# daviyan5/ninpol

Hardware: AMD Instinct MI355X
Metric: Mnodes/s interpolated (GLS, 10M-cell hex mesh) + achieved HBM GB/s vs peak (higher is better)
Workload: dtype f64

## Files before the change

### ninpol_amd/csrc/abi_internal.hpp

```cpp
#pragma once
#include <hip/hip_runtime.h>

#include <algorithm>
#include <chrono>
#include <cstdio>
#include <cstdlib>
#include <initializer_list>
#include <string>
#include <vector>

#include "../../include/ninpol_amd.h"
#include "device_grid.hpp"
#include "grid_host.hpp"
#include "launch.hpp"

struct nin_grid {
    nin::HostGrid h;
    nin::DeviceGrid d;
    std::vector<uint8_t> node_class;
    int coords_dim = 3;
};

#pragma GCC visibility push(hidden)
namespace nin {
// ... 91 lines not shown
};

struct DirtyLaps {
    bool on = getenv("NIN_TIMING") != nullptr;
    hipStream_t stream;
    hipEvent_t e[4] = {nullptr, nullptr, nullptr, nullptr};
    explicit DirtyLaps(hipStream_t s) : stream(s) {}
    ~DirtyLaps() { for (hipEvent_t x : e) if (x) (void)hipEventDestroy(x); }
    void mark(int i) { if (on && !e[i] && hipEventCreate(&e[i]) == hipSuccess) (void)hipEventRecord(e[i], stream); }
    void report(int64_t n) {
        if (!on || !e[0] || !e[1] || !e[2] || !e[3] || hipEventSynchronize(e[3]) != hipSuccess) return;
        float ms[3] = {0.f, 0.f, 0.f};
        for (int i = 0; i < 3; ++i) (void)hipEventElapsedTime(&ms[i], e[i], e[i + 1]);
        fprintf(stderr, "[nin_dirty] nodes %lld compact+readback %.4f descriptors %.4f weights %.4f ms\n", (long long)n, ms[0], ms[1], ms[2]);
    }
};

int build_gls_plan(nin_grid *g);
int gls_only();
int gls_side_begin(DeviceGrid &d, int piece, int add_neumann, double *out, double *nws, hipStream_t stream);
int gls_main(DeviceGrid &d, int piece, bool cube, int only, int add_neumann, double *out, double *nws, hipStream_t stream);
int launch_lists(DeviceGrid &d, int method, const int32_t *lists, const int32_t *off, uint32_t *desc, const size_t *desc_first,
                 int add_neumann, double *out, double *nws, hipStream_t stream, DirtyLaps *laps);
int fetch_flag_bytes(nin_grid *g);
void release_adjoint_state(DeviceGrid &d);

}
#pragma GCC visibility pop
```

### ninpol_amd/csrc/abi_plan.hip

```cpp
#include <hipcub/hipcub.hpp>
#include <cmath>

#include "abi_internal.hpp"
#include "hex8_desc.hpp"
#include "mfw_desc.hpp"
#include "mfg_desc.hpp"
#include "mfx_desc.hpp"
#include "quad4_desc.hpp"

using namespace nin;

namespace {

#ifndef NIN_LOCALITY_RUN
#define NIN_LOCALITY_RUN 16
#endif
constexpr int kLocalityRun = NIN_LOCALITY_RUN;
__device__ __forceinline__ uint32_t spread10(uint32_t v) {
    v = (v | (v << 16)) & 0x030000FFu;
    v = (v | (v << 8)) & 0x0300F00Fu;
    v = (v | (v << 4)) & 0x030C30C3u;
    v = (v | (v << 2)) & 0x09249249u;
    return v;
}
// ... 291 lines not shown
        else if (method == NIN_METHOD_LS) rc = launch_ls(d.v, nullptr, (int32_t)P, (int32_t)g->h.mx_elems_per_point, d.nnz_e, dev_csr_data, dev_neumann_ws, stream);
        else {
            HIP_TRY(hipMemsetAsync(d.gls_queue, 0, kGlsQueueInts * sizeof(int32_t), stream));
            const int only = gls_only();
            if (only < 0) rc = gls_side_begin(d, -1, add_neumann, dev_csr_data, dev_neumann_ws, stream);
            if (!rc) rc = gls_main(d, -1, true, only, add_neumann, dev_csr_data, dev_neumann_ws, stream);
        }
        if (rc) return fail(rc, "kernel launch failed: %s", hipGetErrorString(hipGetLastError()));
        return NIN_OK;
    }
    for (int64_t i = 0; i < n_targets; ++i)
        if (targets[i] < 0 || targets[i] >= P) return fail(NIN_EINVAL, "target %lld out of range", (long long)targets[i]);
    HIP_TRY(hipMemsetAsync(dev_csr_data, 0, (size_t)d.nnz_e * 8, stream));
    HIP_TRY(hipMemsetAsync(dev_neumann_ws, 0, (size_t)P * 8, stream));
    if (n_targets == 0) return NIN_OK;
    const bool gls = method == NIN_METHOD_GLS;
    std::vector<int32_t> lists[kGlsPlanKernels];
    for (int64_t i = 0; i < n_targets; ++i) lists[gls ? gls_class_kernel(g->node_class[targets[i]]) : 0].push_back((int32_t)targets[i]);
    std::vector<int32_t> flat;
    int32_t off[kGlsPlanKernels + 1];
    size_t desc_first[kGlsPlanKernels], words = 0;
    for (int k = 0; k < kGlsPlanKernels; ++k) {
        off[k] = (int32_t)flat.size();
        desc_first[k] = words;
        flat.insert(flat.end(), lists[k].begin(), lists[k].end());
        if (gls) words += lists[k].size() * (size_t)gls_plan_row(k).desc_words;
    }
    off[kGlsPlanKernels] = (int32_t)flat.size();
    DevTmp<int32_t> dl0;
    HIP_TRY(hipMalloc((void **)&dl0, (flat.size() + words) * 4));
    const hipError_t e = hipMemcpy(dl0, flat.data(), flat.size() * 4, hipMemcpyHostToDevice);
    if (e != hipSuccess) return fail(NIN_EHIP, "hipMemcpy: %s", hipGetErrorString(e));
    rc = launch_lists(d, method, dl0, off, reinterpret_cast<uint32_t *>(dl0 + flat.size()), desc_first, add_neumann, dev_csr_data,
                      dev_neumann_ws, stream, nullptr);
    const hipError_t sy = hipStreamSynchronize(stream);
    if (sy != hipSuccess) return fail(NIN_EHIP, "target kernels: %s", hipGetErrorString(sy));
    return rc;
}

int nin_weights_host(nin_grid *g, int method, const int64_t *targets, int64_t n_targets, int add_neumann,
                     double *csr_data, double *neumann_ws) {
    if (!g || !csr_data || !neumann_ws) return fail(NIN_EINVAL, "NULL argument");
    DeviceGrid &d = g->d;
    if (int rc = on_device(g, kHintWeights, false)) return rc;
    HIP_TRY(hipSetDevice(d.device));
    const size_t nb = (size_t)std::max<int64_t>(d.nnz_e, 1) * 8, pb = (size_t)g->h.n_points * 8;
    DevTmp<double> dd, dn;
    HIP_TRY(hipMalloc((void **)&dd, nb));
    hipError_t e = hipMalloc((void **)&dn, pb);
    if (e != hipSuccess) return fail(NIN_ENOMEM, "hipMalloc: %s", hipGetErrorString(e));
    int rc = nin_weights_device(g, method, targets, n_targets, add_neumann, dd, dn, nullptr);
    if (!rc) {
        e = hipDeviceSynchronize();
        if (e == hipSuccess) e = hipMemcpy(csr_data, dd, (size_t)d.nnz_e * 8, hipMemcpyDeviceToHost);
        if (e == hipSuccess) e = hipMemcpy(neumann_ws, dn, pb, hipMemcpyDeviceToHost);
        if (e != hipSuccess) rc = fail(NIN_EHIP, "weights kernel / copy back: %s", hipGetErrorString(e));
// ... 119 lines not shown
```

### ninpol_amd/csrc/abi_update.hip

```cpp
#include <new>

#include "abi_internal.hpp"

using namespace nin;

namespace {

struct GeometryMirror : LazyArrays {
    const DeviceGrid *d;
    explicit GeometryMirror(const DeviceGrid *dg) : d(dg) {}
    template <class T>
    static int get(std::vector<T> &dst, const T *src, size_t n, std::string *err) {
        if (!src) { *err = "the device copy is gone"; return -3; }
        dst.resize(n);
        if (n && hipMemcpy(dst.data(), src, n * sizeof(T), hipMemcpyDeviceToHost) != hipSuccess) { *err = "hipMemcpy (device to host)"; return -3; }
        return 0;
    }
    int fetch(HostGrid &h, unsigned which, std::string *err) override {
        if (d->device < 0 || hipSetDevice(d->device) != hipSuccess) { *err = "the grid has no device copy"; return -3; }
        const size_t P = (size_t)h.n_points, E = (size_t)h.n_elems, F = (size_t)h.n_faces;
        int rc = 0;
        if (!rc && (which & A_COORDS)) rc = get(h.coords, d->v.coords, P * 3, err);
        if (!rc && (which & A_CENTROIDS)) rc = get(h.centroids, d->v.centroids, E * 3, err);
        if (!rc && (which & A_FCENTERS)) rc = get(h.faces_centers, d->v.face_center, F * 3, err);
// ... 344 lines not shown
            else
                snprintf(who, sizeof who, "cell ids outside [0, %lld) were given to nin_fields_scatter_permeability_device", (long long)g->h.n_elems);
            return fail(NIN_EINVAL, "%d %s and written nowhere; nothing was launched, the dirty set is kept", (int)hdr[kDirtyHdrRejected], who);
        }
        d.scattered_cells = d.scattered_nodes = d.scattered_flags = false;
    }
    if (d.all_dirty) {
        if ((rc = nin_weights_device(g, method, nullptr, 0, add_neumann, dev_csr_data, dev_neumann_ws, stream_))) return rc;
        if (clear) {
            if (d.dirty) HIP_TRY(hipMemsetAsync(d.dirty, 0, (size_t)P, stream));
            d.all_dirty = false;
        }
        if (n_recomputed) *n_recomputed = P;
        return NIN_OK;
    }
    const int32_t *off = hdr + kDirtyHdrOffsets;
    const int32_t total = off[kGlsPlanKernels];
    if (total < 0 || total > P) return fail(NIN_EHIP, "the dirty set's lists hold %d nodes of %d", (int)total, (int)P);
    if (n_recomputed) *n_recomputed = total;
    if (total == 0) return NIN_OK;
    size_t desc_first[kGlsPlanKernels], words = 0;
    for (int k = 0; gls && k < kGlsPlanKernels; ++k) {
        if (off[k + 1] < off[k]) return fail(NIN_EHIP, "the dirty set's lists are out of order");
        desc_first[k] = words;
        words += (size_t)(off[k + 1] - off[k]) * (size_t)gls_plan_row(k).desc_words;
    }
    if (words > d.dirty_desc_words && (rc = grow(d, &d.dirty_desc, &d.dirty_desc_words, words + words / 2))) return rc;
    if ((rc = launch_lists(d, method, d.dirty_lists, off, d.dirty_desc, desc_first, add_neumann, dev_csr_data, dev_neumann_ws, stream, &laps)))
        return rc;
    laps.report(total);
    return NIN_OK;
}

int64_t nin_grid_dirty_nodes(nin_grid *g) {
    if (!g || g->d.device < 0 || g->d.prebuilt) return 0;
    DeviceGrid &d = g->d;
    if (d.all_dirty) return -1;
    if (!d.dirty) return 0;
    int32_t n = 0;
    if (hipSetDevice(d.device) != hipSuccess || hipDeviceSynchronize() != hipSuccess ||
        hipMemset(d.dirty_hdr + kDirtyHdrCount, 0, sizeof(int32_t)) != hipSuccess ||
        launch_dirty_count((int32_t)g->h.n_points, d.dirty, d.dirty_hdr + kDirtyHdrCount, nullptr) ||
        hipMemcpy(&n, d.dirty_hdr + kDirtyHdrCount, sizeof n, hipMemcpyDeviceToHost) != hipSuccess) {
        (void)fail(NIN_EHIP, "counting the dirty nodes: %s", hipGetErrorString(hipGetLastError()));
        return -2;
    }
    return n;
// ... 15 lines not shown
```

### ninpol_amd/csrc/gls_plan.hpp

```cpp
#pragma once
#include <cstdint>

#ifdef __HIPCC__
#define NIN_HD __host__ __device__
#else
#define NIN_HD
#endif

namespace nin {

constexpr int kGlsClasses = 5;

constexpr int kGlsPlanKernels = 22;
namespace gk {
enum GlsKernel : int {
    block1, block2, block4, block8, scratch,
    hex8,
    mfw_large, mfw_small, mfw_general,
    small4, small8, small12,
    quad4,
    mfx_6x10, mfx_7x11, mfx_8x13, mfx_9x15, mfx_10x16,
    mfx_boundary,
    mfg_tiles,
    mfx_4x7,
// ... 15 lines not shown

constexpr int kGlsQueueLine = 16;
constexpr int kGlsQueueHex8 = 0, kGlsQueueHex8Lines = 8;
constexpr int kGlsQueueBlock = 1;
constexpr int kGlsQueueMfw = 5;
constexpr int kGlsQueueMfx = 8, kGlsQueueMfxLists = 8;
constexpr int kGlsQueueMfg = 8 * kGlsQueueLine;
constexpr int kGlsQueueInts = 9 * kGlsQueueLine;
static_assert(kGlsQueueBlock > kGlsQueueHex8 && kGlsQueueBlock + (kGlsClasses - 1) <= kGlsQueueMfw, "block counters overlap");
static_assert(kGlsQueueMfw + 3 <= kGlsQueueMfx, "mfw counters overlap the mfx counters");
static_assert(kGlsQueueMfx + kGlsQueueMfxLists <= kGlsQueueLine, "the block / mfw / mfx counters must stay between hex8's ints 0 and 16");
static_assert(kGlsQueueMfg % kGlsQueueLine == 0 && kGlsQueueMfg / kGlsQueueLine >= kGlsQueueHex8 / kGlsQueueLine + kGlsQueueHex8Lines,
              "the mfg counter must lie on none of hex8's eight lines");
static_assert(kGlsQueueMfg < kGlsQueueInts, "the mfg counter lies outside the block");

struct GlsPlanRow {
    GlsFamily family;
    int8_t sub;
    uint8_t class_byte;
    int16_t desc_words;
    int16_t fdq_word;
    int16_t counter;
};
constexpr int kGlsDescHex8 = 4, kGlsDescQuad4 = 2, kGlsDescMfw = 40, kGlsDescMfx = 56, kGlsDescMfg = 124;

NIN_HD constexpr GlsPlanRow gls_plan_row(int k) {
    using F = GlsFamily;
    constexpr GlsPlanRow rows[kGlsPlanKernels] = {
        {F::block,   0,    0,  0,             -1,  kGlsQueueBlock + 0},
        {F::block,   1,    1,  0,             -1,  kGlsQueueBlock + 1},
        {F::block,   2,    2,  0,             -1,  kGlsQueueBlock + 2},
        {F::block,   3,    3,  0,             -1,  kGlsQueueBlock + 3},
        {F::scratch, 4,    4,  0,             -1,  -1},
        {F::hex8,    0,  255,  kGlsDescHex8,  -1,  kGlsQueueHex8},
        {F::mfw,     0,  254,  kGlsDescMfw,   24,  kGlsQueueMfw + 0},
        {F::mfw,     1,  253,  kGlsDescMfw,   24,  kGlsQueueMfw + 1},
        {F::mfw,     2,  252,  kGlsDescMfw,   24,  kGlsQueueMfw + 2},
        {F::small,   0,  249,  0,             -1,  -1},
        {F::small,   1,  250,  0,             -1,  -1},
        {F::small,   2,  251,  0,             -1,  -1},
        {F::quad4,   0,  248,  kGlsDescQuad4, -1,  -1},
        {F::mfx,     0,  243,  kGlsDescMfx,    0,  kGlsQueueMfx + 0},
        {F::mfx,     1,  244,  kGlsDescMfx,    0,  kGlsQueueMfx + 1},
        {F::mfx,     2,  245,  kGlsDescMfx,    0,  kGlsQueueMfx + 2},
        {F::mfx,     3,  246,  kGlsDescMfx,    0,  kGlsQueueMfx + 3},
        {F::mfx,     4,  247,  kGlsDescMfx,    0,  kGlsQueueMfx + 4},
        {F::mfx,     5,  242,  kGlsDescMfx,    0,  kGlsQueueMfx + 5},
// ... 63 lines not shown
```

### ninpol_amd/csrc/grid_device.hip

```cpp
#include <hip/hip_runtime.h>
#include <hipcub/hipcub.hpp>

#include <algorithm>
#include <chrono>
#include <cstdio>
#include <cstdlib>
#include <string>
#include <vector>

#include "device_grid.hpp"
#include "grid_host.hpp"
#include "hex8_desc.hpp"
#include "quad4_desc.hpp"
#include "mfw_desc.hpp"
#include "mfg_desc.hpp"
#include "mfx_desc.hpp"
#include "launch.hpp"

namespace nin {

namespace {

struct Topo {
    int8_t npoel[kNumElementTypes], nfael[kNumElementTypes];
// ... 498 lines not shown
    }
    h.lazy.reset(mir);
    h.have = 0;
    d.prebuilt = true;
    if (getenv("NIN_GRID_EAGER_MIRROR")) {
        if ((rc = h.ensure(A_ALL, err))) return rc;
        lap("to host");
    }
    if (h.build_edges) h.build_inedel();
    return 0;
}

namespace {

__global__ void k_classify(GridView g, int use_group, int force_global, uint8_t *__restrict__ node_class,
                           unsigned long long *__restrict__ class_max) {
    const int64_t p = (int64_t)blockIdx.x * TPB + threadIdx.x;
    if (p >= g.n_points) return;
    const int64_t ne = g.esup_ptr[p + 1] - g.esup_ptr[p], nf = g.fsup_ptr[p + 1] - g.fsup_ptr[p];
    int64_t nbf = 0;
    for (int32_t q = g.fsup_ptr[p]; q < g.fsup_ptr[p + 1]; ++q) nbf += g.face_cells[2 * (int64_t)g.fsup[q] + 1] == -1;
    if ((use_group & kRouteHex8) && ne == 8 && nf == 12 && nbf == 0 && g.dim == 3) {
        int32_t d[4];
        if (hex8_descriptor(g, (int32_t)p, d)) { node_class[p] = gls_class_byte(gk::hex8); return; }
    }
    const bool small_fits = (use_group & kRouteSmall) && !force_global && g.dim == 3 && ne <= 12 && nf <= 48 && ne + 3 * nf <= 64;
    if ((use_group & kRouteMfw) && nbf == 0 && ne <= kMfwMaxCells) {
        uint32_t w[kMfwDescWords];
        const int kind = mfw_descriptor(g, (int32_t)p, w);
        if (kind == 1) {
            const int F = w[24] & 255, D = (w[24] >> 8) & 255;
            node_class[p] = (F <= kMfwSmallFronts && D <= kMfwSmallDense) ? gls_class_byte(gk::mfw_small) : gls_class_byte(gk::mfw_large);
            return;
        }
        if (kind == 2 && (use_group & kRouteMfwGeneral) && !small_fits && !(use_group & kRouteMfxTakesGeneral)) { node_class[p] = gls_class_byte(gk::mfw_general); return; }
    }
    const bool small_fits_b = (use_group & kRouteSmall) && !force_global && g.dim == 3 && ne <= 12 && nf <= 48 && ne + 3 * (nf - nbf) + nbf <= 64;
    const bool small_class_candidate = (use_group & kRouteMfxSmall) && nbf == 0 && small_fits && ne >= 9;
    if ((use_group & kRouteMfx) && !force_global && ne <= kMfxMaxCells && (!(nbf == 0 ? small_fits : small_fits_b) || small_class_candidate) &&
        (nbf == 0 || !(use_group & kRouteMfxNoBoundary))) {
        uint32_t w[kMfxDescWords];
        const int k = mfx_descriptor(g, (int32_t)p, w);
        if (k == kMfxSmallCode && (use_group & kRouteMfxSmall)) { node_class[p] = gls_class_byte(gk::mfx_4x7); return; }
        if (k == kMfxMidCode && (use_group & kRouteMfx7x12)) { node_class[p] = gls_class_byte(gk::mfx_7x12); return; }
        if (k > 0 && nbf == 0 && !small_fits) { node_class[p] = (uint8_t)(gls_class_byte(gk::mfx_6x10) + (k == kMfxSmallCode ? 1 : k == kMfxMidCode ? 3 : k) - 1); return; }
        if (k > 0 && k <= 2 && nbf > 0) { node_class[p] = gls_class_byte(gk::mfx_boundary); return; }
    }
// ... 31 lines not shown
```

### ninpol_amd/csrc/hex8_desc.hpp

```cpp
#pragma once
#include <cstdint>

#include "device_grid.hpp"

namespace nin {

constexpr int kHex8DescWords = 4;

#ifdef __HIPCC__
__device__ inline bool hex8_descriptor(const GridView &g, int32_t p, int32_t d[kHex8DescWords]) {
    const int32_t eb = g.esup_ptr[p], fb = g.fsup_ptr[p];
    if (g.esup_ptr[p + 1] - eb != 8 || g.fsup_ptr[p + 1] - fb != 12 || g.dim != 3) return false;
    int32_t cells[8];
    for (int i = 0; i < 8; ++i) cells[i] = g.esup[eb + i];
    uint32_t adj[8] = {0, 0, 0, 0, 0, 0, 0, 0};
    int deg[8] = {0, 0, 0, 0, 0, 0, 0, 0};
    for (int fi = 0; fi < 12; ++fi) {
        const int64_t f = g.fsup[fb + fi];
        const int32_t a = g.face_cells[2 * f], b = g.face_cells[2 * f + 1];
        if (b < 0) return false;
        int ia = -1, ib = -1;
        for (int i = 0; i < 8; ++i) {
            ia = cells[i] == a ? i : ia;
            ib = cells[i] == b ? i : ib;
        }
        if (ia < 0 || ib < 0 || ia == ib || deg[ia] >= 3 || deg[ib] >= 3) return false;
        adj[ia] |= (uint32_t)(fi | (ib << 4) | (1 << 7)) << (8 * deg[ia]);
        adj[ib] |= (uint32_t)(fi | (ia << 4)) << (8 * deg[ib]);
        ++deg[ia];
        ++deg[ib];
    }
    for (int i = 0; i < 8; ++i)
        if (deg[i] != 3) return false;
// ... 17 lines not shown
    for (int i = 0, l = 0; i < 8; ++i)
        if (color[i] == 0) even[l++] = i;
    for (int l = 0; l < 4; ++l) {
        const int e = even[l];
        unsigned seen = 0;
        for (int k = 0; k < 3; ++k) seen |= 1u << ((adj[e] >> (8 * k + 4)) & 7);
        int missing = -1, n_missing = 0;
        for (int i = 0; i < 8; ++i)
            if (color[i] == 1 && !((seen >> i) & 1)) { missing = i; ++n_missing; }
        if (n_missing != 1 || oslot[missing] >= 0) return false;
        oslot[missing] = 3 - l;
        odd[3 - l] = missing;
    }
    for (int l = 0; l < 4; ++l) {
        const int e = even[l];
        uint32_t w = (uint32_t)e | ((uint32_t)odd[l] << 3);
        int ord[3] = {0, 1, 2};
        for (int x = 0; x < 2; ++x)
            for (int y = 0; y < 2 - x; ++y) {
                const int sa = oslot[(adj[e] >> (8 * ord[y] + 4)) & 7], sb = oslot[(adj[e] >> (8 * ord[y + 1] + 4)) & 7];
                if (sa > sb) { const int t = ord[y]; ord[y] = ord[y + 1]; ord[y + 1] = t; }
            }
        for (int i = 0; i < 3; ++i) w |= ((adj[e] >> (8 * ord[i])) & 0xFFu) << (6 + 8 * i);
        d[l] = (int32_t)w;
    }
    return true;
}
#endif

}
```

### ninpol_amd/csrc/kernels_gls_hex8mf.hip

```cpp
#include <hip/hip_runtime.h>

#include <cstdio>
#include <cstdlib>

#include "device_grid.hpp"
#include "gls_device_math.hpp"
#include "hex8_desc.hpp"
#include "launch.hpp"

namespace nin {

namespace {

using namespace glsmath;

__device__ __forceinline__ double quad_sum(double v) {
    v += dpp_mov<0xB1>(v);
    v += dpp_mov<0x4E>(v);
    return v;
}
template <int L>
__device__ __forceinline__ double quad_bcast(double v) { return dpp_mov<L * 0x55>(v); }

constexpr int NPW = 16;
// ... 3 lines not shown
struct BackLoop {
    static __device__ __forceinline__ void run(const double (&C)[NR][NC], const double (&rinvq)[3], double (&t)[3],
                                               double (&y)[12], int l) {
        constexpr int Q = K / 4, LAM = K % 4;
        const double yk = quad_bcast<LAM>(t[Q] * rinvq[Q]);
        y[K] = yk;
#pragma unroll
        for (int q = 0; q < Q; ++q) t[q] = fma(-C[q][K], yk, t[q]);
        if (LAM > 0) t[Q] = fma((l < LAM) ? -C[Q][K] : 0.0, yk, t[Q]);
        BackLoop<K - 1>::run(C, rinvq, t, y, l);
    }
};
template <>
struct BackLoop<-1> {
    static __device__ __forceinline__ void run(const double (&)[NR][NC], const double (&)[3], double (&)[3], double (&)[12], int) {}
};

#ifdef NIN_W2_FENCE_COLUMNS
#define NIN_W2_COLUMN_FENCE() __builtin_amdgcn_sched_barrier(0)
#else
#define NIN_W2_COLUMN_FENCE() do { } while (0)
#endif
constexpr int W2_SLOTS = 35;
constexpr int W2_WAVE_DOUBLES = W2_SLOTS * 64 + NPW * 8 + 64;

template <int K>
__device__ __forceinline__ void p2_step_lean(double (&C)[NR][NC], double (&rinvq)[3], int l) {
    constexpr int Q = K / 4, LAM = K % 4;
    const bool is_piv = (l == LAM);
    const double xq = (l > LAM) ? C[Q][K] : 0.0;
    double ss = xq * xq;
#pragma unroll
    for (int r = Q + 1; r < NR; ++r) ss = fma(C[r][K], C[r][K], ss);
    ss = quad_sum(ss);
    const double alpha = quad_bcast<LAM>(C[Q][K]);
    const House h = house_unguarded(alpha, ss);
    rinvq[Q] = is_piv ? h.rinv : rinvq[Q];
    const double vq = is_piv ? h.vp : xq;
#pragma unroll
    for (int j = K + 1; j < NC; ++j) {
        double a = vq * C[Q][j];
#pragma unroll
        for (int r = Q + 1; r < NR; ++r) a = fma(C[r][K], C[r][j], a);
        const double w = -(h.g * quad_sum(a));
        C[Q][j] = fma(w, vq, C[Q][j]);
#pragma unroll
        for (int r = Q + 1; r < NR; ++r) C[r][j] = fma(w, C[r][K], C[r][j]);
// ... 19 lines not shown
        w0 = -(g3[0] * P[0][0]);
        w1 = -(g3[1] * (w0 * cc[0]));
        w2 = -(g3[2] * fma(w1, cc[2], w0 * cc[1]));
    } else {
        w0 = -(g3[0] * fma(P[R0 + 2][0], b[2], fma(P[R0 + 1][0], b[1], P[R0][0] * b[0])));
        w1 = -(g3[1] * fma(w0, cc[0], fma(P[R0 + 2][1], b[2], fma(P[R0 + 1][1], b[1], P[R0][1] * b[0]))));
        const double d2 = (R0 >= 2) ? fma(P[R0 + 2][2], b[2], fma(P[R0 + 1][2], b[1], P[R0 < 0 ? 0 : R0][2] * b[0]))
                                    : fma(P[R0 + 2][2], b[2], P[R0 + 1][2] * b[1]);
        w2 = -(g3[2] * fma(w1, cc[2], fma(w0, cc[1], d2)));
    }
    double ub;
    if (R0 < 0) ub = fma(q[0], w0, z[0]);
    else if (R0 == 1) ub = fma(q[0], w0, fma(z[2], b[1], z[1] * b[0]));
    else ub = q[0] * w0;
    u_out = fma(q[2], w2, fma(q[1], w1, ub));
#pragma unroll
    for (int r = 3; r < 10; ++r) {
        const bool own = R0 >= 0 && r >= R0 && r < R0 + 3;
        const double v = own ? fma(w0, P[r][0], b[own ? r - R0 : 0]) : w0 * P[r][0];
        fill[r - 3] = fma(w2, P[r][2], fma(w1, P[r][1], v));
    }
}

__device__ __forceinline__ void w2_dma(const void *gptr, uint32_t *row) {
    __builtin_amdgcn_global_load_lds((const __attribute__((address_space(1))) void *)gptr, (__attribute__((address_space(3))) void *)row, 4, 0, 0);
}
__device__ __forceinline__ void w2_dma_wait() {
    __builtin_amdgcn_sched_barrier(0);
    asm volatile("s_waitcnt vmcnt(0)" ::: "memory");
    __builtin_amdgcn_sched_barrier(0);
}
__device__ __forceinline__ void w2_stage_a(const int32_t *nodes, const int32_t *desc, int32_t wg, int32_t count, int nd, int l,
                                           uint32_t *row_p, uint32_t *row_dsc) {
    const int32_t idx = wg * NPW + nd;
    const uint32_t sel = (uint32_t)((idx >= 0 && idx < count) ? idx : count - 1);
    w2_dma(nodes + sel, row_p);
    w2_dma(desc + 4 * (size_t)sel + l, row_dsc);
}
__device__ __forceinline__ void w2_stage_b(const GridView &g, uint32_t p, uint32_t *rows_b) {
    w2_dma(g.esup_ptr + p, rows_b);
    w2_dma(g.fsup_ptr + p, rows_b + 64);
}
__device__ __forceinline__ void w2_stage_c(const GridView &g, uint32_t p, uint32_t eb, uint32_t fb, uint32_t dsc, uint32_t *rows_n) {
    const uint32_t *xw = reinterpret_cast<const uint32_t *>(g.coords) + 6 * (size_t)p;
#pragma unroll
    for (int k = 0; k < 6; ++k) w2_dma(xw + k, rows_n + 64 * (2 + k));
    w2_dma(g.esup + eb + (dsc & 7), rows_n + 64 * 8);
    w2_dma(g.esup + eb + ((dsc >> 3) & 7), rows_n + 64 * 9);
#pragma unroll
    for (int i = 0; i < 3; ++i) w2_dma(g.fsup + fb + ((dsc >> (6 + 8 * i)) & 15), rows_n + 64 * (10 + i));
}
struct W2Geo {
    double Ke[9], dme, ce[3];
    double Ko[9], dmo, co[3];
    double fc[3][3];
    float fn[3][3];
    uint32_t flags;
};
__device__ __forceinline__ void w2_stage_d(const GridView &g, const uint32_t *row_p, const uint32_t *rows_n, int lane, W2Geo &q) {
    q.flags = g.flags[row_p[lane]];
    const uint32_t ce = rows_n[64 * 8 + lane], co = rows_n[64 * 9 + lane];
#pragma unroll
    for (int k = 0; k < 9; ++k) { q.Ke[k] = g.perm[9 * (size_t)ce + k]; q.Ko[k] = g.perm[9 * (size_t)co + k]; }
    q.dme = g.diff_mag[ce];
    q.dmo = g.diff_mag[co];
#pragma unroll
    for (int t = 0; t < 3; ++t) { q.ce[t] = g.centroids[3 * (size_t)ce + t]; q.co[t] = g.centroids[3 * (size_t)co + t]; }
#pragma unroll
    for (int i = 0; i < 3; ++i) {
        const uint32_t f = rows_n[64 * (10 + i) + lane];
#pragma unroll
        for (int t = 0; t < 3; ++t) { q.fn[i][t] = g.face_normal[3 * (size_t)f + t]; q.fc[i][t] = g.face_center[3 * (size_t)f + t]; }
    }
}
template <int I>
__device__ __forceinline__ double w2_across(double v) { return dpp_mov<I == 0 ? 0x40 : I == 1 ? 0xA5 : 0xFE>(v); }

#ifndef W2_C_STEP
#define W2_C_STEP 0
#endif
#ifndef W2_D_STEP
#define W2_D_STEP 6
#endif
static_assert(W2_C_STEP >= 0 && W2_C_STEP < W2_D_STEP && W2_D_STEP <= 12, "level 2 before level 3, both in phase 2");

#ifdef NIN_W2_TRACE
__device__ unsigned long long nin_w2_trace[4096 * 4];
#endif
template <bool APPLY>
__global__ __launch_bounds__(256, 2) void nin_gls_hex8w2_kernel(GridView g, const int32_t *__restrict__ nodes,
                                                                const int32_t *__restrict__ desc, int32_t count,
                                                                int add_neumann, double *__restrict__ out,
                                                                double *__restrict__ nws, int32_t *__restrict__ queue,
                                                                const double *__restrict__ u_cells, int32_t n_fields,
                                                                double *__restrict__ values) {
    __shared__ double lds_all[4][W2_WAVE_DOUBLES];
    __shared__ double tau_tab[TAU_TAB_DOUBLES];
    static_assert(2 * (sizeof(double) * (4 * W2_WAVE_DOUBLES + TAU_TAB_DOUBLES)) <= 160 * 1024, "two workgroups per CU");
    tau_table_to_lds(tau_tab);
    __syncthreads();
    const lds_cdouble_ptr tau_lds = (lds_cdouble_ptr)tau_tab;
    const int lane = threadIdx.x & 63, wave = threadIdx.x >> 6;
    const int l = lane & 3, nd = lane >> 2;
    double *const L = lds_all[wave] + lane;
    double *const wbuf = lds_all[wave] + W2_SLOTS * 64;
    uint32_t *const row_p = reinterpret_cast<uint32_t *>(lds_all[wave] + W2_SLOTS * 64 + NPW * 8);
    uint32_t *const row_dsc = row_p + 64;
    uint32_t *const rows_b = reinterpret_cast<uint32_t *>(wbuf);
    uint32_t *const rows_n = reinterpret_cast<uint32_t *>(lds_all[wave] + 13 * 64);

    const int32_t n_groups = (count + NPW - 1) / NPW;
    int32_t wg_lo, wg_end;
    int32_t *q;
    if ((gridDim.x & 7) == 0) {
        const int32_t xcd = blockIdx.x & 7, per = (n_groups + 7) / 8;
        wg_lo = xcd * per;
        wg_end = (xcd + 1) * per < n_groups ? (xcd + 1) * per : n_groups;
        q = queue + kGlsQueueLine * xcd;
    } else {
        wg_lo = 0;
        wg_end = n_groups;
        q = queue;
    }
    int32_t ticket = 0;
    if (lane == 0) ticket = atomicAdd(q, 1);
    int32_t wg = wg_lo + __builtin_amdgcn_readfirstlane(ticket);
    if (lane == 0) ticket = atomicAdd(q, 1);
    int32_t wg_next = wg_lo + __builtin_amdgcn_readfirstlane(ticket);
    W2Geo geo;
    w2_stage_a(nodes, desc, wg, count, nd, l, row_p, row_dsc);
    w2_dma_wait();
    w2_stage_b(g, row_p[lane], rows_b);
    w2_dma_wait();
    {
        const uint32_t eb0 = rows_b[lane];
        rows_n[lane] = eb0;
        w2_stage_c(g, row_p[lane], eb0, rows_b[64 + lane], row_dsc[lane], rows_n);
    }
    w2_dma_wait();
    w2_stage_d(g, row_p, rows_n, lane, geo);
#ifdef NIN_MF_STAMPS
#ifndef NIN_MF_STAMP_PASS
#define NIN_MF_STAMP_PASS 8
#endif
    unsigned long long stamps[8];
    int n_stamp = 0, pass_no = 0;
#define NIN_MF_STAMP() do { if (n_stamp < 8) { __builtin_amdgcn_sched_barrier(0); stamps[n_stamp++] = __builtin_amdgcn_s_memtime(); __builtin_amdgcn_s_waitcnt(0xC07F); __builtin_amdgcn_sched_barrier(0); } } while (0)
#else
#define NIN_MF_STAMP() do { } while (0)
#endif
#ifdef NIN_W2_TRACE
    const unsigned long long trace_t0 = __builtin_amdgcn_s_memrealtime();
    unsigned trace_passes = 0;
#endif
    while (wg < wg_end) {
#ifdef NIN_W2_TRACE
        ++trace_passes;
#endif
#ifdef NIN_MF_STAMPS
        n_stamp = 0;
#endif
        NIN_MF_STAMP();
        const bool valid = wg * NPW + nd < count;
        __builtin_amdgcn_s_waitcnt(0x0F70);
#ifdef NIN_MF_STAMP_SPLIT
        NIN_MF_STAMP();
#define NIN_MF_STAMP_BACK() do { } while (0)
#else
#define NIN_MF_STAMP_BACK() NIN_MF_STAMP()
#endif
        const uint32_t p = row_p[lane], dsc = row_dsc[lane], eb = rows_n[lane];
        double xv[3];
#pragma unroll
        for (int k = 0; k < 3; ++k) xv[k] = __hiloint2double((int)rows_n[64 * (3 + 2 * k) + lane], (int)rows_n[64 * (2 + 2 * k) + lane]);
        const bool is_neu = (geo.flags & 2) != 0;
        __builtin_amdgcn_s_waitcnt(0xC07F);
        w2_stage_a(nodes, desc, wg_next, count, nd, l, row_p, row_dsc);
        __builtin_amdgcn_sched_barrier(0);

        double P[10][3], de[3], dod[3], nb0[3][3], sav[3][2][3];
        {
            const double dme = geo.dme;
#pragma unroll
            for (int t = 0; t < 3; ++t) {
                de[t] = geo.ce[t] - xv[t];
                dod[t] = geo.co[t] - xv[t];
                P[0][t] = de[t];
            }
#pragma unroll
            for (int i = 0; i < 3; ++i) {
                const uint32_t w = dsc >> (6 + 8 * i);
                const double N0 = (double)geo.fn[i][0], N1 = (double)geo.fn[i][1], N2 = (double)geo.fn[i][2];
                const double T0 = xv[0] - geo.fc[i][0], T1 = xv[1] - geo.fc[i][1], T2 = xv[2] - geo.fc[i][2];
                const double U0 = N1 * T2 - N2 * T1, U1 = N2 * T0 - N0 * T2, U2 = N0 * T1 - N1 * T0;
                auto across = [&](double v) { return i == 0 ? w2_across<0>(v) : i == 1 ? w2_across<1>(v) : w2_across<2>(v); };
                const double dmn = across(geo.dmo);
                double eta = 0.0;
                eta = dme > eta ? dme : eta;
                eta = dmn > eta ? dmn : eta;
                const double tj = face_tau_tab_t<true>(U0 * U0 + U1 * U1 + U2 * U2, eta, tau_lds);
                const bool side_a = ((w >> 7) & 1) != 0;
                const double sg = side_a ? -1.0 : 1.0;
                double Kn[9];
#pragma unroll
                for (int k = 0; k < 9; ++k) Kn[k] = across(geo.Ko[k]);
#pragma unroll
                for (int t = 0; t < 3; ++t) {
                    P[1 + 3 * i][t] = sg * (geo.Ke[t * 3 + 0] * N0 + geo.Ke[t * 3 + 1] * N1 + geo.Ke[t * 3 + 2] * N2);
                    nb0[i][t] = -sg * (Kn[t * 3 + 0] * N0 + Kn[t * 3 + 1] * N1 + Kn[t * 3 + 2] * N2);
                }
                sav[i][0][0] = sg * T0; sav[i][0][1] = sg * T1; sav[i][0][2] = sg * T2;
                sav[i][1][0] = sg * (tj * U0); sav[i][1][1] = sg * (tj * U1); sav[i][1][2] = sg * (tj * U2);
#pragma unroll
                for (int t = 0; t < 3; ++t) { P[2 + 3 * i][t] = sav[i][0][t]; P[3 + 3 * i][t] = sav[i][1][t]; }
            }
        }
#pragma unroll
        for (int r = 0; r < 10; ++r) { pin(P[r][0]); pin(P[r][1]); pin(P[r][2]); }
#pragma unroll
        for (int i = 0; i < 3; ++i) { pin(nb0[i][0]); pin(nb0[i][1]); pin(nb0[i][2]); }
        NIN_MF_STAMP();
#ifndef W2_B_LATE
        w2_dma_wait();
        w2_stage_b(g, row_p[lane], rows_b);
#endif
        if (lane == 0) ticket = atomicAdd(q, 1);
        __builtin_amdgcn_sched_barrier(0);
        double C[NR][NC];
        double u[9], se, F1[7][2], F2[7][3];
        {
            double g3[3], z[3];
            front_panel(P, de, g3, z);
            pin(z[0]); pin(z[1]); pin(z[2]);
            double cc[3];
            cc[0] = P[1][1] * P[1][0];
            cc[1] = P[2][2] * P[2][0];
            cc[2] = P[2][2] * P[2][1];
#pragma unroll
            for (int r = 2; r < 10; ++r) cc[0] = fma(P[r][1], P[r][0], cc[0]);
#pragma unroll
            for (int r = 3; r < 10; ++r) { cc[1] = fma(P[r][2], P[r][0], cc[1]); cc[2] = fma(P[r][2], P[r][1], cc[2]); }
            double q3[3];
            q3[0] = fma(z[2], P[2][0], fma(z[1], P[1][0], z[0] * P[0][0]));
            q3[1] = fma(z[2], P[2][1], z[1] * P[1][1]);
            q3[2] = z[2] * P[2][2];
            {
                const double none[3] = {0.0, 0.0, 0.0};
                double fill[7];
// ... 23 lines not shown
                if (t == 0) {
#pragma unroll
                    for (int r = 0; r < 7; ++r) L[64 * (28 + r)] = fill[r];
                } else {
#pragma unroll
                    for (int r = 0; r < 7; ++r) F1[r][t - 1] = fill[r];
                }
                NIN_W2_COLUMN_FENCE();
            }
            __builtin_amdgcn_sched_barrier(0);
#pragma unroll
            for (int t = 0; t < 3; ++t) {
                const double b[3] = {nb0[2][t], -sav[2][0][t], -sav[2][1][t]};
                double fill[7];
                w2_column<7>(P, g3, cc, z, q3, b, u[6 + t], fill);
                pin(u[6 + t]);
#pragma unroll
                for (int r = 0; r < 7; ++r) F2[r][t] = fill[r];
                NIN_W2_COLUMN_FENCE();
            }
            __builtin_amdgcn_sched_barrier(0);
        }
        NIN_MF_STAMP();
#ifdef W2_B_LATE
        w2_dma_wait();
        w2_stage_b(g, row_p[lane], rows_b);
#endif
        {
            const bool lt3 = l < 3, lt2 = l < 2, eq0 = l == 0, ge2 = l >= 2, ge1 = l >= 1, eq3 = l == 3;
#pragma unroll
            for (int t = 0; t < 3; ++t) {
#pragma unroll
                for (int r = 0; r < 7; ++r) {
                    const double f1 = (t == 0) ? L[64 * (28 + r)] : F1[r][t == 0 ? 0 : t - 1];
                    const double f0 = L[64 * (7 + 7 * t + r)];
                    C[r][6 + t] = eq0 ? F2[r][t] : (ge2 ? f1 : 0.0);
                    C[r][9 + t] = ge1 ? F2[r][t] : 0.0;
                    C[r][3 + t] = lt2 ? f1 : (eq3 ? f0 : 0.0);
                    C[r][t] = lt3 ? f0 : 0.0;
                }
            }
#pragma unroll
            for (int r = 0; r < 7; ++r) C[r][12] = L[64 * r];
        }
        __builtin_amdgcn_sched_barrier(0);
#pragma unroll
        for (int j = 0; j < 9; ++j) L[64 * j] = u[j];
        L[64 * 9] = se;
#pragma unroll
        for (int s = 0; s < 4; ++s) {
#pragma unroll
            for (int t = 0; t < 3; ++t) C[7][3 * s + t] = (l == s) ? dod[t] : 0.0;
        }
        C[7][12] = 1.0;
        __builtin_amdgcn_sched_barrier(0);

        double rinvq[3] = {0.0, 0.0, 0.0};
        NIN_MF_STAMP();
        __builtin_amdgcn_sched_barrier(0);
        P2LeanLoop<0, W2_C_STEP>::run(C, rinvq, l);
        __builtin_amdgcn_sched_barrier(0);
        w2_dma_wait();
        {
            const uint32_t ebn = rows_b[lane];
            rows_n[lane] = ebn;
            w2_stage_c(g, row_p[lane], ebn, rows_b[64 + lane], row_dsc[lane], rows_n);
        }
        __builtin_amdgcn_sched_barrier(0);
        P2LeanLoop<W2_C_STEP, W2_D_STEP>::run(C, rinvq, l);
        NIN_MF_STAMP();
        __builtin_amdgcn_sched_barrier(0);
        w2_dma_wait();
        int32_t wg_after = wg_lo + __builtin_amdgcn_readfirstlane(ticket);
        asm volatile("" : "+s"(wg_after));
        __builtin_amdgcn_sched_barrier(0);
        w2_stage_d(g, row_p, rows_n, lane, geo);
        __builtin_amdgcn_sched_barrier(0);
        P2LeanLoop<W2_D_STEP, 12>::run(C, rinvq, l);
        NIN_MF_STAMP();
        double y[12], t3[3] = {C[0][12], C[1][12], C[2][12]};
        BackLoop<11>::run(C, rinvq, t3, y, l);
        NIN_MF_STAMP_BACK();
        double tail = 0.0;
#pragma unroll
        for (int r = 3; r < NR; ++r) tail = fma(C[r][12], C[r][12], tail);
        const double rr = quad_sum(tail);

        double re = 1.0 - L[64 * 9];
#pragma unroll
        for (int i = 0; i < 3; ++i) {
            const bool low = i < 3 - l;
#pragma unroll
            for (int t = 0; t < 3; ++t) re = fma(L[64 * (3 * i + t)], low ? y[3 * i + t] : y[3 * i + 3 + t], re);
        }
        double dots[4];
#pragma unroll
        for (int s = 0; s < 4; ++s) dots[s] = fma(dod[2], y[3 * s + 2], fma(dod[1], y[3 * s + 1], dod[0] * y[3 * s]));
        const double dsel = (l == 0) ? dots[0] : (l == 1) ? dots[1] : (l == 2) ? dots[2] : dots[3];
        const double ro = 1.0 - dsel;
// ... 26 lines not shown
        NIN_MF_STAMP();
#ifdef NIN_MF_STAMPS
        if (blockIdx.x == 0 && threadIdx.x == 0 && ++pass_no == NIN_MF_STAMP_PASS)
            for (int i = 0; i < 8; ++i) nws[nodes[i]] = (double)(stamps[i] - stamps[0]);
#endif
        wg = wg_next;
        wg_next = wg_after;
    }
    w2_dma_wait();
#ifdef NIN_W2_TRACE
    if (lane == 0 && blockIdx.x < 1024) {
        unsigned long long *t = nin_w2_trace + 4 * ((size_t)blockIdx.x * 4 + wave);
        t[0] = trace_t0;
        t[1] = __builtin_amdgcn_s_memrealtime();
        t[2] = __builtin_amdgcn_s_getreg((4 << 0) | (0 << 6) | (31 << 11));
        t[3] = trace_passes;
    }
#endif
}

__global__ void k_hex8_desc(GridView g, const int32_t *__restrict__ nodes, int32_t count, int32_t *__restrict__ desc) {
    const int64_t i = (int64_t)blockIdx.x * blockDim.x + threadIdx.x;
    if (i >= count) return;
    int32_t d[4] = {0, 0, 0, 0};
    (void)hex8_descriptor(g, nodes ? nodes[i] : (int32_t)i, d);
#pragma unroll
    for (int l = 0; l < 4; ++l) desc[4 * i + l] = d[l];
}

}

int launch_hex8_desc(const GridView &g, const int32_t *nodes, int32_t count, int32_t *desc, hipStream_t stream) {
    if (count <= 0) return 0;
    hipLaunchKernelGGL(k_hex8_desc, dim3((unsigned)((count + 255) / 256)), dim3(256), 0, stream, g, nodes, count, desc);
    return hipGetLastError() == hipSuccess ? 0 : -3;
}

int launch_gls_hex8mf(const GridView &g, const int32_t *nodes, const int32_t *desc, int32_t count, int add_neumann,
                      double *out, double *nws, int32_t *queue, hipStream_t stream) {
    if (count <= 0) return 0;
    int64_t blocks = ((int64_t)count + 4 * NPW - 1) / (4 * NPW);
    const char *cap_env = getenv("NIN_W2_BLOCKS");
    const int64_t cap2 = cap_env ? atoll(cap_env) : 512;
    if (blocks > cap2) blocks = cap2;
    if (blocks > 8) blocks &= ~(int64_t)7;
    if (getenv("NIN_DEBUG_OCCUPANCY") != nullptr) {
        int nb = -1;
        (void)hipOccupancyMaxActiveBlocksPerMultiprocessor(&nb, nin_gls_hex8w2_kernel<false>, 256, 0);
        fprintf(stderr, "nin_gls_hex8w2_kernel: %d workgroups per CU, %lld launched\n", nb, (long long)blocks);
    }
// ... 34 lines not shown
```

Baseline: 2226.

## Precompute per-lane hex8 records to collapse dependent index loads into one prefetch

The hex8 descriptor kernel now writes an 8-word record per lane: node id, esup offset, the two cell ids, the three face ids and the packed word. The matrix-free GLS kernel fetches this record with two 16-byte global-to-LDS DMAs instead of a multi-stage chain (nodes/desc, then esup_ptr/fsup_ptr, then coords/esup/fsup). This removes two dependent latency rounds and several staging waits inside the per-node loop. In exchange each descriptor grows from 4 to 32 words per node, which adds HBM traffic, and coordinates are now read directly from global memory in stage d. Descriptor offsets are aligned to 4 words so the 16-byte loads stay aligned.

```diff
diff --git a/ninpol_amd/csrc/abi_internal.hpp b/ninpol_amd/csrc/abi_internal.hpp
--- a/ninpol_amd/csrc/abi_internal.hpp
+++ b/ninpol_amd/csrc/abi_internal.hpp
@@ -137,6 +137,7 @@
 int gls_main(DeviceGrid &d, int piece, bool cube, int only, int add_neumann, double *out, double *nws, hipStream_t stream);
 int launch_lists(DeviceGrid &d, int method, const int32_t *lists, const int32_t *off, uint32_t *desc, const size_t *desc_first,
                  int add_neumann, double *out, double *nws, hipStream_t stream, DirtyLaps *laps);
+inline size_t desc_align(size_t words) { return (words + 3) & ~(size_t)3; }
 int fetch_flag_bytes(nin_grid *g);
 void release_adjoint_state(DeviceGrid &d);
 
diff --git a/ninpol_amd/csrc/abi_plan.hip b/ninpol_amd/csrc/abi_plan.hip
--- a/ninpol_amd/csrc/abi_plan.hip
+++ b/ninpol_amd/csrc/abi_plan.hip
@@ -337,16 +337,17 @@
     size_t desc_first[kGlsPlanKernels], words = 0;
     for (int k = 0; k < kGlsPlanKernels; ++k) {
         off[k] = (int32_t)flat.size();
-        desc_first[k] = words;
+        desc_first[k] = words = desc_align(words);
         flat.insert(flat.end(), lists[k].begin(), lists[k].end());
         if (gls) words += lists[k].size() * (size_t)gls_plan_row(k).desc_words;
     }
     off[kGlsPlanKernels] = (int32_t)flat.size();
+    const size_t list_words = desc_align(flat.size());
     DevTmp<int32_t> dl0;
-    HIP_TRY(hipMalloc((void **)&dl0, (flat.size() + words) * 4));
+    HIP_TRY(hipMalloc((void **)&dl0, (list_words + words) * 4));
     const hipError_t e = hipMemcpy(dl0, flat.data(), flat.size() * 4, hipMemcpyHostToDevice);
     if (e != hipSuccess) return fail(NIN_EHIP, "hipMemcpy: %s", hipGetErrorString(e));
-    rc = launch_lists(d, method, dl0, off, reinterpret_cast<uint32_t *>(dl0 + flat.size()), desc_first, add_neumann, dev_csr_data,
+    rc = launch_lists(d, method, dl0, off, reinterpret_cast<uint32_t *>(dl0 + list_words), desc_first, add_neumann, dev_csr_data,
                       dev_neumann_ws, stream, nullptr);
     const hipError_t sy = hipStreamSynchronize(stream);
     if (sy != hipSuccess) return fail(NIN_EHIP, "target kernels: %s", hipGetErrorString(sy));
diff --git a/ninpol_amd/csrc/abi_update.hip b/ninpol_amd/csrc/abi_update.hip
--- a/ninpol_amd/csrc/abi_update.hip
+++ b/ninpol_amd/csrc/abi_update.hip
@@ -390,7 +390,7 @@
     size_t desc_first[kGlsPlanKernels], words = 0;
     for (int k = 0; gls && k < kGlsPlanKernels; ++k) {
         if (off[k + 1] < off[k]) return fail(NIN_EHIP, "the dirty set's lists are out of order");
-        desc_first[k] = words;
+        desc_first[k] = words = desc_align(words);
         words += (size_t)(off[k + 1] - off[k]) * (size_t)gls_plan_row(k).desc_words;
     }
     if (words > d.dirty_desc_words && (rc = grow(d, &d.dirty_desc, &d.dirty_desc_words, words + words / 2))) return rc;
diff --git a/ninpol_amd/csrc/gls_plan.hpp b/ninpol_amd/csrc/gls_plan.hpp
--- a/ninpol_amd/csrc/gls_plan.hpp
+++ b/ninpol_amd/csrc/gls_plan.hpp
@@ -61,7 +61,7 @@
     int16_t fdq_word;
     int16_t counter;
 };
-constexpr int kGlsDescHex8 = 4, kGlsDescQuad4 = 2, kGlsDescMfw = 40, kGlsDescMfx = 56, kGlsDescMfg = 124;
+constexpr int kGlsDescHex8 = 32, kGlsDescQuad4 = 2, kGlsDescMfw = 40, kGlsDescMfx = 56, kGlsDescMfg = 124;
 
 NIN_HD constexpr GlsPlanRow gls_plan_row(int k) {
     using F = GlsFamily;
diff --git a/ninpol_amd/csrc/grid_device.hip b/ninpol_amd/csrc/grid_device.hip
--- a/ninpol_amd/csrc/grid_device.hip
+++ b/ninpol_amd/csrc/grid_device.hip
@@ -544,7 +544,7 @@
     for (int32_t q = g.fsup_ptr[p]; q < g.fsup_ptr[p + 1]; ++q) nbf += g.face_cells[2 * (int64_t)g.fsup[q] + 1] == -1;
     if ((use_group & kRouteHex8) && ne == 8 && nf == 12 && nbf == 0 && g.dim == 3) {
         int32_t d[4];
-        if (hex8_descriptor(g, (int32_t)p, d)) { node_class[p] = gls_class_byte(gk::hex8); return; }
+        if (hex8_descriptor<false>(g, (int32_t)p, d)) { node_class[p] = gls_class_byte(gk::hex8); return; }
     }
     const bool small_fits = (use_group & kRouteSmall) && !force_global && g.dim == 3 && ne <= 12 && nf <= 48 && ne + 3 * nf <= 64;
     if ((use_group & kRouteMfw) && nbf == 0 && ne <= kMfwMaxCells) {
diff --git a/ninpol_amd/csrc/hex8_desc.hpp b/ninpol_amd/csrc/hex8_desc.hpp
--- a/ninpol_amd/csrc/hex8_desc.hpp
+++ b/ninpol_amd/csrc/hex8_desc.hpp
@@ -5,10 +5,12 @@
 
 namespace nin {
 
-constexpr int kHex8DescWords = 4;
+constexpr int kHex8LaneWords = 8;
+constexpr int kHex8DescWords = 4 * kHex8LaneWords;
 
 #ifdef __HIPCC__
-__device__ inline bool hex8_descriptor(const GridView &g, int32_t p, int32_t d[kHex8DescWords]) {
+template <bool RECORD>
+__device__ inline bool hex8_descriptor(const GridView &g, int32_t p, int32_t *d) {
     const int32_t eb = g.esup_ptr[p], fb = g.fsup_ptr[p];
     if (g.esup_ptr[p + 1] - eb != 8 || g.fsup_ptr[p + 1] - fb != 12 || g.dim != 3) return false;
     int32_t cells[8];
@@ -72,7 +74,17 @@
                 if (sa > sb) { const int t = ord[y]; ord[y] = ord[y + 1]; ord[y + 1] = t; }
             }
         for (int i = 0; i < 3; ++i) w |= ((adj[e] >> (8 * ord[i])) & 0xFFu) << (6 + 8 * i);
-        d[l] = (int32_t)w;
+        if (RECORD) {
+            int32_t *r = d + kHex8LaneWords * l;
+            r[0] = p;
+            r[1] = eb;
+            r[2] = g.esup[eb + e];
+            r[3] = g.esup[eb + odd[l]];
+            for (int i = 0; i < 3; ++i) r[4 + i] = g.fsup[fb + ((w >> (6 + 8 * i)) & 15)];
+            r[7] = (int32_t)w;
+        } else {
+            d[l] = (int32_t)w;
+        }
     }
     return true;
 }
diff --git a/ninpol_amd/csrc/kernels_gls_hex8mf.hip b/ninpol_amd/csrc/kernels_gls_hex8mf.hip
--- a/ninpol_amd/csrc/kernels_gls_hex8mf.hip
+++ b/ninpol_amd/csrc/kernels_gls_hex8mf.hip
@@ -49,7 +49,7 @@
 #define NIN_W2_COLUMN_FENCE() do { } while (0)
 #endif
 constexpr int W2_SLOTS = 35;
-constexpr int W2_WAVE_DOUBLES = W2_SLOTS * 64 + NPW * 8 + 64;
+constexpr int W2_WAVE_DOUBLES = W2_SLOTS * 64 + NPW * 8;
 
 template <int K>
 __device__ __forceinline__ void p2_step_lean(double (&C)[NR][NC], double (&rinvq)[3], int l) {
@@ -115,44 +115,37 @@
     }
 }
 
-__device__ __forceinline__ void w2_dma(const void *gptr, uint32_t *row) {
-    __builtin_amdgcn_global_load_lds((const __attribute__((address_space(1))) void *)gptr, (__attribute__((address_space(3))) void *)row, 4, 0, 0);
+__device__ __forceinline__ void w2_dma16(const void *gptr, uint32_t *row) {
+    __builtin_amdgcn_global_load_lds((const __attribute__((address_space(1))) void *)gptr, (__attribute__((address_space(3))) void *)row, 16, 0, 0);
 }
 __device__ __forceinline__ void w2_dma_wait() {
     __builtin_amdgcn_sched_barrier(0);
     asm volatile("s_waitcnt vmcnt(0)" ::: "memory");
     __builtin_amdgcn_sched_barrier(0);
 }
-__device__ __forceinline__ void w2_stage_a(const int32_t *nodes, const int32_t *desc, int32_t wg, int32_t count, int nd, int l,
-                                           uint32_t *row_p, uint32_t *row_dsc) {
+constexpr int W2_REC_ROW = 256;
+__device__ __forceinline__ void w2_stage_rec(const int32_t *rec, int32_t wg, int32_t count, int nd, int l, uint32_t *rows_r) {
     const int32_t idx = wg * NPW + nd;
     const uint32_t sel = (uint32_t)((idx >= 0 && idx < count) ? idx : count - 1);
-    w2_dma(nodes + sel, row_p);
-    w2_dma(desc + 4 * (size_t)sel + l, row_dsc);
-}
-__device__ __forceinline__ void w2_stage_b(const GridView &g, uint32_t p, uint32_t *rows_b) {
-    w2_dma(g.esup_ptr + p, rows_b);
-    w2_dma(g.fsup_ptr + p, rows_b + 64);
-}
-__device__ __forceinline__ void w2_stage_c(const GridView &g, uint32_t p, uint32_t eb, uint32_t fb, uint32_t dsc, uint32_t *rows_n) {
-    const uint32_t *xw = reinterpret_cast<const uint32_t *>(g.coords) + 6 * (size_t)p;
-#pragma unroll
-    for (int k = 0; k < 6; ++k) w2_dma(xw + k, rows_n + 64 * (2 + k));
-    w2_dma(g.esup + eb + (dsc & 7), rows_n + 64 * 8);
-    w2_dma(g.esup + eb + ((dsc >> 3) & 7), rows_n + 64 * 9);
-#pragma unroll
-    for (int i = 0; i < 3; ++i) w2_dma(g.fsup + fb + ((dsc >> (6 + 8 * i)) & 15), rows_n + 64 * (10 + i));
+    const int32_t *r = rec + kHex8LaneWords * (4 * (size_t)sel + l);
+    w2_dma16(r, rows_r);
+    w2_dma16(r + 4, rows_r + W2_REC_ROW);
 }
 struct W2Geo {
     double Ke[9], dme, ce[3];
     double Ko[9], dmo, co[3];
     double fc[3][3];
     float fn[3][3];
+    double xv[3];
     uint32_t flags;
 };
-__device__ __forceinline__ void w2_stage_d(const GridView &g, const uint32_t *row_p, const uint32_t *rows_n, int lane, W2Geo &q) {
-    q.flags = g.flags[row_p[lane]];
-    const uint32_t ce = rows_n[64 * 8 + lane], co = rows_n[64 * 9 + lane];
+__device__ __forceinline__ void w2_stage_d(const GridView &g, const uint32_t *rows_r, int lane, W2Geo &q) {
+    const uint4 ra = *reinterpret_cast<const uint4 *>(rows_r + 4 * lane);
+    const uint4 rb = *reinterpret_cast<const uint4 *>(rows_r + W2_REC_ROW + 4 * lane);
+#pragma unroll
+    for (int t = 0; t < 3; ++t) q.xv[t] = g.coords[3 * (size_t)ra.x + t];
+    q.flags = g.flags[ra.x];
+    const uint32_t ce = ra.z, co = ra.w;
 #pragma unroll
     for (int k = 0; k < 9; ++k) { q.Ke[k] = g.perm[9 * (size_t)ce + k]; q.Ko[k] = g.perm[9 * (size_t)co + k]; }
     q.dme = g.diff_mag[ce];
@@ -161,7 +154,7 @@
     for (int t = 0; t < 3; ++t) { q.ce[t] = g.centroids[3 * (size_t)ce + t]; q.co[t] = g.centroids[3 * (size_t)co + t]; }
 #pragma unroll
     for (int i = 0; i < 3; ++i) {
-        const uint32_t f = rows_n[64 * (10 + i) + lane];
+        const uint32_t f = i == 0 ? rb.x : i == 1 ? rb.y : rb.z;
 #pragma unroll
         for (int t = 0; t < 3; ++t) { q.fn[i][t] = g.face_normal[3 * (size_t)f + t]; q.fc[i][t] = g.face_center[3 * (size_t)f + t]; }
     }
@@ -169,13 +162,10 @@
 template <int I>
 __device__ __forceinline__ double w2_across(double v) { return dpp_mov<I == 0 ? 0x40 : I == 1 ? 0xA5 : 0xFE>(v); }
 
-#ifndef W2_C_STEP
-#define W2_C_STEP 0
-#endif
 #ifndef W2_D_STEP
 #define W2_D_STEP 6
 #endif
-static_assert(W2_C_STEP >= 0 && W2_C_STEP < W2_D_STEP && W2_D_STEP <= 12, "level 2 before level 3, both in phase 2");
+static_assert(W2_D_STEP >= 0 && W2_D_STEP <= 12, "the geometry is requested in phase 2");
 
 #ifdef NIN_W2_TRACE
 __device__ unsigned long long nin_w2_trace[4096 * 4];
@@ -187,7 +177,8 @@
                                                                 double *__restrict__ nws, int32_t *__restrict__ queue,
                                                                 const double *__restrict__ u_cells, int32_t n_fields,
                                                                 double *__restrict__ values) {
-    __shared__ double lds_all[4][W2_WAVE_DOUBLES];
+    __shared__ __attribute__((aligned(16))) double lds_all[4][W2_WAVE_DOUBLES];
+    static_assert(W2_WAVE_DOUBLES % 2 == 0, "a wave's slots begin on a 16-byte boundary (the records' rows)");
     __shared__ double tau_tab[TAU_TAB_DOUBLES];
     static_assert(2 * (sizeof(double) * (4 * W2_WAVE_DOUBLES + TAU_TAB_DOUBLES)) <= 160 * 1024, "two workgroups per CU");
     tau_table_to_lds(tau_tab);
@@ -197,10 +188,7 @@
     const int l = lane & 3, nd = lane >> 2;
     double *const L = lds_all[wave] + lane;
     double *const wbuf = lds_all[wave] + W2_SLOTS * 64;
-    uint32_t *const row_p = reinterpret_cast<uint32_t *>(lds_all[wave] + W2_SLOTS * 64 + NPW * 8);
-    uint32_t *const row_dsc = row_p + 64;
-    uint32_t *const rows_b = reinterpret_cast<uint32_t *>(wbuf);
-    uint32_t *const rows_n = reinterpret_cast<uint32_t *>(lds_all[wave] + 13 * 64);
+    uint32_t *const rows_r = reinterpret_cast<uint32_t *>(lds_all[wave] + 13 * 64);
 
     const int32_t n_groups = (count + NPW - 1) / NPW;
     int32_t wg_lo, wg_end;
@@ -221,17 +209,9 @@
     if (lane == 0) ticket = atomicAdd(q, 1);
     int32_t wg_next = wg_lo + __builtin_amdgcn_readfirstlane(ticket);
     W2Geo geo;
-    w2_stage_a(nodes, desc, wg, count, nd, l, row_p, row_dsc);
+    w2_stage_rec(desc, wg, count, nd, l, rows_r);
     w2_dma_wait();
-    w2_stage_b(g, row_p[lane], rows_b);
-    w2_dma_wait();
-    {
-        const uint32_t eb0 = rows_b[lane];
-        rows_n[lane] = eb0;
-        w2_stage_c(g, row_p[lane], eb0, rows_b[64 + lane], row_dsc[lane], rows_n);
-    }
-    w2_dma_wait();
-    w2_stage_d(g, row_p, rows_n, lane, geo);
+    w2_stage_d(g, rows_r, lane, geo);
 #ifdef NIN_MF_STAMPS
 #ifndef NIN_MF_STAMP_PASS
 #define NIN_MF_STAMP_PASS 8
@@ -262,13 +242,10 @@
 #else
 #define NIN_MF_STAMP_BACK() NIN_MF_STAMP()
 #endif
-        const uint32_t p = row_p[lane], dsc = row_dsc[lane], eb = rows_n[lane];
-        double xv[3];
-#pragma unroll
-        for (int k = 0; k < 3; ++k) xv[k] = __hiloint2double((int)rows_n[64 * (3 + 2 * k) + lane], (int)rows_n[64 * (2 + 2 * k) + lane]);
+        uint32_t p = rows_r[4 * lane], eb = rows_r[4 * lane + 1], dsc = rows_r[W2_REC_ROW + 4 * lane + 3];
+        asm volatile("" : "+v"(p), "+v"(eb), "+v"(dsc));
+        const double xv[3] = {geo.xv[0], geo.xv[1], geo.xv[2]};
         const bool is_neu = (geo.flags & 2) != 0;
-        __builtin_amdgcn_s_waitcnt(0xC07F);
-        w2_stage_a(nodes, desc, wg_next, count, nd, l, row_p, row_dsc);
         __builtin_amdgcn_sched_barrier(0);
 
         double P[10][3], de[3], dod[3], nb0[3][3], sav[3][2][3];
@@ -308,15 +285,7 @@
                 for (int t = 0; t < 3; ++t) { P[2 + 3 * i][t] = sav[i][0][t]; P[3 + 3 * i][t] = sav[i][1][t]; }
             }
         }
-#pragma unroll
-        for (int r = 0; r < 10; ++r) { pin(P[r][0]); pin(P[r][1]); pin(P[r][2]); }
-#pragma unroll
-        for (int i = 0; i < 3; ++i) { pin(nb0[i][0]); pin(nb0[i][1]); pin(nb0[i][2]); }
-        NIN_MF_STAMP();
-#ifndef W2_B_LATE
-        w2_dma_wait();
-        w2_stage_b(g, row_p[lane], rows_b);
-#endif
+        NIN_MF_STAMP();
         if (lane == 0) ticket = atomicAdd(q, 1);
         __builtin_amdgcn_sched_barrier(0);
         double C[NR][NC];
@@ -386,10 +355,6 @@
             __builtin_amdgcn_sched_barrier(0);
         }
         NIN_MF_STAMP();
-#ifdef W2_B_LATE
-        w2_dma_wait();
-        w2_stage_b(g, row_p[lane], rows_b);
-#endif
         {
             const bool lt3 = l < 3, lt2 = l < 2, eq0 = l == 0, ge2 = l >= 2, ge1 = l >= 1, eq3 = l == 3;
 #pragma unroll
@@ -422,23 +387,17 @@
         double rinvq[3] = {0.0, 0.0, 0.0};
         NIN_MF_STAMP();
         __builtin_amdgcn_sched_barrier(0);
-        P2LeanLoop<0, W2_C_STEP>::run(C, rinvq, l);
-        __builtin_amdgcn_sched_barrier(0);
-        w2_dma_wait();
-        {
-            const uint32_t ebn = rows_b[lane];
-            rows_n[lane] = ebn;
-            w2_stage_c(g, row_p[lane], ebn, rows_b[64 + lane], row_dsc[lane], rows_n);
-        }
-        __builtin_amdgcn_sched_barrier(0);
-        P2LeanLoop<W2_C_STEP, W2_D_STEP>::run(C, rinvq, l);
+        __builtin_amdgcn_s_waitcnt(0xC07F);
+        w2_stage_rec(desc, wg_next, count, nd, l, rows_r);
+        __builtin_amdgcn_sched_barrier(0);
+        P2LeanLoop<0, W2_D_STEP>::run(C, rinvq, l);
         NIN_MF_STAMP();
         __builtin_amdgcn_sched_barrier(0);
         w2_dma_wait();
         int32_t wg_after = wg_lo + __builtin_amdgcn_readfirstlane(ticket);
         asm volatile("" : "+s"(wg_after));
         __builtin_amdgcn_sched_barrier(0);
-        w2_stage_d(g, row_p, rows_n, lane, geo);
+        w2_stage_d(g, rows_r, lane, geo);
         __builtin_amdgcn_sched_barrier(0);
         P2LeanLoop<W2_D_STEP, 12>::run(C, rinvq, l);
         NIN_MF_STAMP();
@@ -511,10 +470,11 @@
 __global__ void k_hex8_desc(GridView g, const int32_t *__restrict__ nodes, int32_t count, int32_t *__restrict__ desc) {
     const int64_t i = (int64_t)blockIdx.x * blockDim.x + threadIdx.x;
     if (i >= count) return;
-    int32_t d[4] = {0, 0, 0, 0};
-    (void)hex8_descriptor(g, nodes ? nodes[i] : (int32_t)i, d);
-#pragma unroll
-    for (int l = 0; l < 4; ++l) desc[4 * i + l] = d[l];
+    int32_t d[kHex8DescWords] = {};
+    (void)hex8_descriptor<true>(g, nodes ? nodes[i] : (int32_t)i, d);
+    int4 *rec = reinterpret_cast<int4 *>(desc) + (kHex8DescWords / 4) * i;
+#pragma unroll
+    for (int w = 0; w < kHex8DescWords / 4; ++w) rec[w] = make_int4(d[4 * w], d[4 * w + 1], d[4 * w + 2], d[4 * w + 3]);
 }
 
 }
```

New measurement: 2270 (median of 6 runs). 1.02x the previous value.
